# Joao-M-Silva/padel_analytics

Measured on AMD Instinct MI355X. Metric: frames/sec (all trackers) on 1280x720, higher is better.
Workload: dtype f32-equivalent (h2: fp16 pairs h + m/2048, 2 or 3 f16 MFMA products per multiply, fp32 accumulate)

## Files before the change

### padel_analytics_amd/csrc/engine.cpp

```cpp
#include "../../include/padel_hip.h"
#include "kernels.h"
#include <rccl/rccl.h>

#include <algorithm>
#include <cmath>
#include <cstdio>
#include <cstdlib>
#include <cstring>
#include <dlfcn.h>
#include <map>
#include <string>
#include <vector>

using namespace padel;

static thread_local std::string g_err;

struct Tuning {
    int impl = 2;
    int variant = -1;
    int tune = 1;
    int tap_pd = 2;
    int graph = 0;
    int timeline = 0;
    int alias = 1;
    int fuse_stem = 1;
    int w_single = 1;
    int fuse_sppf = 1;
    int fold_up = 1;
};

struct pa_comm;

struct pa_engine {
    int dev = 0;
    hipStream_t stream = nullptr;
    hipStream_t copy_stream = nullptr;
    std::string err;
    bool profiling = false;
    float* zeros = nullptr;
    Tuning t;
    int tuning_epoch = 0;
    std::string timeline_path;
    pa_comm* comm = nullptr;
};

static int env_int(const char* k, int dflt) { const char* v = getenv(k); return v ? atoi(v) : dflt; }

#define PA_FAIL(eng, ...)                                        \
    do {                                                         \
        char _b[512];                                            \
        snprintf(_b, sizeof(_b), __VA_ARGS__);                   \
        if (eng) (eng)->err = _b; else g_err = _b;               \
        return 1;                                                \
    } while (0)

#define PA_HIP(eng, call)                                                                  \
    do {                                                                                   \
        hipError_t _e = (call);                                                            \
        if (_e != hipSuccess) {                                                            \
            (void)hipGetLastError();    \
            PA_FAIL(eng, "%s failed: %s (%s:%d)", #call, hipGetErrorString(_e), __FILE__, __LINE__); \
        }                                                                                  \
    } while (0)

struct ProfRec { int kind; int ksize; double flops; hipEvent_t e0, e1; float ms; int M, cout, cin, stride, mf, nf, res; int tile; const char* family; };

struct pa_model {
    pa_engine* e = nullptr;
    pa_model_desc d{};
    std::vector<pa_buf_desc> bufs;
    std::vector<pa_op_desc> ops;
    std::vector<int> fold_src;
    std::vector<int> fold_dst;
    float* d_w = nullptr;
    size_t n_w = 0;
    char* d_wr = nullptr;
    std::vector<long long> wr_off;
    bool wr_valid = false;
    unsigned* d_ovf = nullptr;
    float* d_stage = nullptr; size_t stage_cap = 0;
    float* d_fc = nullptr;
    int fc_nout = 0;
    int max_batch = 64;

    bool planned = false;
    int p_h0 = 0, p_w0 = 0, p_imgsz = 0, p_pre = 0, p_auto = 0, p_batch = 0;
    int net_h = 0, net_w = 0;
    int rw = 0, rh = 0, top = 0, left = 0, lb_mode = 0;
    std::vector<float*> bptr;
    void* arena = nullptr;
    size_t arena_bytes = 0, logical_bytes = 0;
    unsigned h_ovf = 0;
    bool ovf_cached = false;
    unsigned* h_pin = nullptr;
    hipEvent_t tk_ev[PA_MAX_INFLIGHT]{};
    bool tk_busy[PA_MAX_INFLIGHT]{};
    int next_ticket = 0, n_inflight = 0;
    std::vector<int32_t> classes_host;
    std::map<int, hipGraphExec_t> graphs;
    int graph_epoch = -1;
    uint8_t* d_frames = nullptr; size_t frames_cap = 0;
    uint8_t* d_netin = nullptr;
    uint8_t* d_tmp = nullptr;
    int32_t *d_xtab = nullptr, *d_ytab = nullptr;
    int32_t *d_hb = nullptr, *d_hk = nullptr, *d_vb = nullptr, *d_vk = nullptr;
    int hks = 0, vks = 0;
    int A = 0, P2 = 0;
    HeadLevel lv[3]{};
    float* d_cand = nullptr; int32_t* d_cidx = nullptr; int32_t* d_ccnt = nullptr;
    uint64_t* d_keys = nullptr; int32_t* d_order = nullptr; uint8_t* d_supp = nullptr;
    float* d_oboxes = nullptr; float* d_okpts = nullptr; int32_t* d_ocnt = nullptr;
    int32_t* d_classes = nullptr; int classes_cap = 0;
    int last_n = 0;
    std::vector<ProfRec> prof;
    size_t n_prof = 0;
};

static void find_upsample_folds(pa_model* m);

extern "C" {

int pa_abi_version(void) { return PA_ABI_VERSION; }

int pa_device_count(void) {
    int n = 0;
    if (hipGetDeviceCount(&n) != hipSuccess) return 0;
    return n;
}

const char* pa_last_error(pa_engine* eng) { return eng ? eng->err.c_str() : g_err.c_str(); }

int pa_engine_create(int device_id, pa_engine** out) {
    if (!out) PA_FAIL((pa_engine*)nullptr, "pa_engine_create: out is NULL");
    int n = 0;
    PA_HIP((pa_engine*)nullptr, hipGetDeviceCount(&n));
    if (device_id < 0 || device_id >= n) PA_FAIL((pa_engine*)nullptr, "pa_engine_create: device %d of %d", device_id, n);
    PA_HIP((pa_engine*)nullptr, hipSetDevice(device_id));
    pa_engine* e = new pa_engine();
    e->dev = device_id;
    hipError_t r = hipStreamCreateWithFlags(&e->stream, hipStreamNonBlocking);
    if (r != hipSuccess) { delete e; PA_FAIL((pa_engine*)nullptr, "hipStreamCreate: %s", hipGetErrorString(r)); }
    if (r == hipSuccess) r = hipStreamCreateWithFlags(&e->copy_stream, hipStreamNonBlocking);
    if (r != hipSuccess) { delete e; PA_FAIL((pa_engine*)nullptr, "hipStreamCreate: %s", hipGetErrorString(r)); }
    r = hipMalloc((void**)&e->zeros, 256);
    if (r == hipSuccess) r = hipMemset(e->zeros, 0, 256);
    if (r != hipSuccess) { delete e; PA_FAIL((pa_engine*)nullptr, "zero page: %s", hipGetErrorString(r)); }
    r = padel::init_misc_kernels();
    if (r != hipSuccess) { delete e; PA_FAIL((pa_engine*)nullptr, "kernel attributes: %s", hipGetErrorString(r)); }
    if (const char* v = getenv("PADEL_CONV_IMPL")) {
        if (v[0] == 'l') { delete e; PA_FAIL((pa_engine*)nullptr, "PADEL_CONV_IMPL=%s: the LDS kernel was retired in round 5; tap or bx3", v); }
        e->t.impl = (v[0] == 'b') ? 2 : 0;
    }
    e->t.variant = env_int("PADEL_CONV_VARIANT", -1);
    e->t.tune = env_int("PADEL_CONV_TUNE", 1);
    e->t.tap_pd = env_int("PADEL_CONV_TAP_PD", 2) == 3 ? 3 : 2;
    e->t.graph = env_int("PADEL_GRAPH", 0);
    e->t.fuse_stem = env_int("PADEL_FUSE_STEM", 1);
    e->t.fuse_sppf = env_int("PADEL_FUSE_SPPF", 1);
    e->t.alias = env_int("PADEL_ALIAS", 1);
    e->t.fold_up = env_int("PADEL_FOLD_UP", 1);
    *out = e;
    return 0;
}

int pa_engine_set_tuning(pa_engine* e, const char* key, int value) {
    if (!e || !key) return 1;
    const std::string k = key;
    if (k == "impl") {
        if (value != 0 && value != 2) PA_FAIL(e, "tuning impl = %d: 0 (fp32-input MFMA tap kernels) or 2 (bf16x3); 1 was the LDS kernel, retired in round 5 (tools/legacy_conv)", value);
        e->t.impl = value;
    }
    else if (k == "variant") e->t.variant = value;
    else if (k == "tune") e->t.tune = value;
    else if (k == "tap_pd") e->t.tap_pd = (value == 3) ? 3 : 2;
    else if (k == "graph") e->t.graph = value ? 1 : 0;
    else if (k == "timeline") e->t.timeline = value ? 1 : 0;
    else if (k == "alias") e->t.alias = value ? 1 : 0;
    else if (k == "fold_up") e->t.fold_up = value ? 1 : 0;
    else if (!strcmp(key, "fuse_stem")) e->t.fuse_stem = value;
    else if (!strcmp(key, "fuse_sppf")) e->t.fuse_sppf = value;
    else if (!strcmp(key, "w_single")) e->t.w_single = value ? 1 : 0;
    else PA_FAIL(e, "pa_engine_set_tuning: unknown key '%s'", key);
    e->tuning_epoch++;
    return 0;
}

int pa_engine_set_timeline_path(pa_engine* e, const char* path) {
    if (!e) return 1;
    e->timeline_path = path ? path : "";
    return 0;
}

void pa_engine_destroy(pa_engine* e) {
    if (!e) return;
    hipSetDevice(e->dev);
    pa_engine_comm_destroy(e);
    if (e->zeros) hipFree(e->zeros);
    if (e->stream) hipStreamDestroy(e->stream);
    if (e->copy_stream) hipStreamDestroy(e->copy_stream);
    delete e;
}

int pa_engine_synchronize(pa_engine* e) {
    PA_HIP(e, hipSetDevice(e->dev));
    PA_HIP(e, hipStreamSynchronize(e->stream));
    return 0;
}

int pa_engine_set_profiling(pa_engine* e, int enable) { e->profiling = enable != 0; return 0; }

int pa_device_malloc(pa_engine* e, size_t nbytes, void** out) {
    PA_HIP(e, hipSetDevice(e->dev));
    PA_HIP(e, hipMalloc(out, nbytes));
    return 0;
}
int pa_device_free(pa_engine* e, void* p) {
    PA_HIP(e, hipSetDevice(e->dev));
    PA_HIP(e, hipFree(p));
    return 0;
}
int pa_memcpy_h2d(pa_engine* e, void* dst, const void* src, size_t n) {
    PA_HIP(e, hipSetDevice(e->dev));
    PA_HIP(e, hipMemcpyAsync(dst, src, n, hipMemcpyHostToDevice, e->stream));
    PA_HIP(e, hipStreamSynchronize(e->stream));
    return 0;
}
int pa_upload(pa_engine* e, void* dst, const void* src, size_t n) {
    PA_HIP(e, hipSetDevice(e->dev));
    PA_HIP(e, hipMemcpyAsync(dst, src, n, hipMemcpyHostToDevice, e->copy_stream));
    PA_HIP(e, hipStreamSynchronize(e->copy_stream));
    return 0;
}
int pa_host_register(pa_engine* e, void* ptr, size_t nbytes) {
    PA_HIP(e, hipSetDevice(e->dev));
    PA_HIP(e, hipHostRegister(ptr, nbytes, hipHostRegisterDefault));
    return 0;
}
int pa_host_unregister(pa_engine* e, void* ptr) {
    PA_HIP(e, hipSetDevice(e->dev));
    PA_HIP(e, hipHostUnregister(ptr));
    return 0;
}
int pa_memcpy_d2h(pa_engine* e, void* dst, const void* src, size_t n) {
    PA_HIP(e, hipSetDevice(e->dev));
    PA_HIP(e, hipMemcpyAsync(dst, src, n, hipMemcpyDeviceToHost, e->stream));
    PA_HIP(e, hipStreamSynchronize(e->stream));
    return 0;
}

static int validate_desc(pa_engine* e, const pa_model_desc* d, size_t n_floats) {
    if (d->n_bufs <= 0 || d->n_ops <= 0 || !d->bufs || !d->ops) PA_FAIL(e, "model desc: empty graph");
    const bool f16 = d->dtype == PA_DTYPE_F16, h2 = d->dtype == PA_DTYPE_H2;
    if (d->dtype != PA_DTYPE_F32 && d->dtype != PA_DTYPE_F16 && d->dtype != PA_DTYPE_H2) PA_FAIL(e, "model desc: dtype %d", d->dtype);
    const int kalign = f16 ? 31 : 15, valign = f16 ? 7 : 3;
    for (int i = 0; i < d->n_bufs; ++i)
        if (d->bufs[i].level < 0 || d->bufs[i].level > 6 || d->bufs[i].channels <= 0 || (d->bufs[i].channels & 3))
            PA_FAIL(e, "model desc: buffer %d (level %d, channels %d)", i, d->bufs[i].level, d->bufs[i].channels);
    auto okslice = [&](int b, int off, int c) {
        return b >= 0 && b < d->n_bufs && off >= 0 && c > 0 && off + c <= d->bufs[b].channels;
    };
    auto is_head_buf = [&](int b) { return b == d->head_buf[0] || b == d->head_buf[1] || b == d->head_buf[2]; };
    if (h2)
        for (int i = 0; i < d->n_bufs; ++i)
// ... 419 lines not shown
    return 0;
}

static ProfRec* prof_begin(pa_model* m, size_t idx, int kind, int ksize, double flops) {
    if (!m->e->profiling) return nullptr;
    if (m->prof.size() <= idx) {
        m->prof.resize(idx + 1);
        hipEventCreate(&m->prof[idx].e0);
        hipEventCreate(&m->prof[idx].e1);
    }
    ProfRec* r = &m->prof[idx];
    r->kind = kind; r->ksize = ksize; r->flops = flops; r->ms = 0.f;
    r->M = r->cout = r->cin = r->stride = r->mf = r->nf = r->res = 0;
    r->tile = -1; r->family = "";
    hipEventRecord(r->e0, m->e->stream);
    return r;
}
static void prof_end(pa_model* m, ProfRec* r) { if (r) hipEventRecord(r->e1, m->e->stream); }

static int conv_launch_args(const pa_model* m, size_t i, int n, ConvArgs& a) {
    const pa_engine* e = m->e;
    const pa_op_desc& o = m->ops[i];
    const pa_buf_desc& ob = m->bufs[o.out_buf];
    const pa_buf_desc& ib = m->bufs[o.in_buf];
    const int Ho = m->net_h >> ob.level, Wo = m->net_w >> ob.level;
    a.in = m->bptr[o.in_buf]; a.in_cs = ib.channels; a.in_choff = o.in_choff;
    a.out = m->bptr[o.out_buf]; a.out_cs = ob.channels; a.out_choff = o.out_choff;
    a.res = o.res_buf >= 0 ? m->bptr[o.res_buf] : nullptr;
    a.res_cs = o.res_buf >= 0 ? m->bufs[o.res_buf].channels : 0; a.res_choff = o.res_choff;
    a.res_pre = (o.res_buf >= 0 && (o.flags & PA_CONV_RES_PREACT)) ? 1 : 0;
    a.zeros = e->zeros;
    a.w = m->d_w + o.w_off; a.bias = m->d_w + o.b_off;
    a.H = m->net_h >> ib.level; a.W = m->net_w >> ib.level; a.Ho = Ho; a.Wo = Wo;
    a.cin = o.cin; a.cout = o.cout; a.n16 = o.npad / 16; a.ksize = o.ksize; a.stride = o.stride; a.act = o.act;
    a.M = n * Ho * Wo;
    fill_fastdiv((unsigned)(Ho * Wo), &a.howo_magic, &a.howo_shift);
    fill_fastdiv((unsigned)Wo, &a.wo_magic, &a.wo_shift);
    a.tune = e->t.tune; a.tap_pd = e->t.tap_pd;
    const bool f16 = m->d.dtype == PA_DTYPE_F16, h2 = m->d.dtype == PA_DTYPE_H2;
    const bool use_tap = e->t.impl == 0 || f16;
    const bool use_bx3 = !f16 && !h2 && e->t.impl == 2 && o.reserved > 0;
    a.w3 = use_bx3 ? (const void*)(m->d_w + o.reserved) : nullptr;
    a.out_f32 = (f16 || h2) && (o.out_buf == m->d.head_buf[0] || o.out_buf == m->d.head_buf[1] || o.out_buf == m->d.head_buf[2]);
    if (h2) {
        a.oscale = m->d_w + o.reserved;
        a.ovf_flag = m->d_ovf;
        a.w_single = (o.flags & PA_CONV_W_SINGLE) && e->t.w_single ? 1 : 0;
        a.wr = (m->wr_valid && i < m->wr_off.size() && m->wr_off[i] >= 0) ? (const void*)(m->d_wr + m->wr_off[i]) : nullptr;
        const int lv = e->t.variant >= 0 ? e->t.variant : choose_conv_h2_variant(a);
        if (fold_active(m, (int)i) && (o.ksize == 1 || (lv >= 300 && lv < 400 && conv_h2p_supported(a)))) {
            const pa_op_desc& u = m->ops[m->fold_src[i]];
            a.in2 = m->bptr[u.in_buf]; a.in2_cs = m->bufs[u.in_buf].channels; a.in2_choff = u.in_choff; a.up_c = u.cin;
        }
        return lv;
    }
    const int lv = e->t.variant >= 0 ? e->t.variant
                   : f16 ? choose_conv_tap16_variant(a)
                   : use_bx3 ? choose_conv_bx3_variant(a)
                         : choose_conv_tap_variant(a.M, a.n16);
    if (use_bx3 && fold_active(m, (int)i) && (o.ksize == 1 || (lv >= 300 && lv < 400 && conv_bx3p_supported(a)))) {
        const pa_op_desc& u = m->ops[m->fold_src[i]];
        a.in2 = m->bptr[u.in_buf]; a.in2_cs = m->bufs[u.in_buf].channels; a.in2_choff = u.in_choff; a.up_c = u.cin;
    }
    return lv;
}

static bool stem_fusable(const pa_model* m, size_t i) {
    if (i + 1 >= m->ops.size()) return false;
    const pa_op_desc& st = m->ops[i];
    const pa_op_desc& c = m->ops[i + 1];
    if (c.kind != PA_OP_CONV || c.ksize != 3 || c.stride != 2 || c.in_buf != st.out_buf || c.in_choff != st.out_choff || c.cin != st.cout ||
        c.res_buf >= 0)
        return false;
    for (int l = 0; l < 3; ++l) if (m->d.head_buf[l] == st.out_buf) return false;
    for (size_t k = 0; k < m->ops.size(); ++k) {
        if (k == i || k == i + 1) continue;
        const pa_op_desc& o = m->ops[k];
        if (o.kind != PA_OP_STEM && o.in_buf == st.out_buf) return false;
        if (o.kind == PA_OP_CONV && o.res_buf == st.out_buf) return false;
    }
    return true;
}

static int run_ops(pa_model* m, int n, size_t* pi) {
    pa_engine* e = m->e;
    hipStream_t s = e->stream;
    for (size_t i = 0; i < m->ops.size(); ++i) {
        const pa_op_desc& o = m->ops[i];
        const pa_buf_desc& ob = m->bufs[o.out_buf];
        const int Ho = m->net_h >> ob.level, Wo = m->net_w >> ob.level;
        hipError_t r = hipSuccess;
        ProfRec* pr = nullptr;
        if (o.kind == PA_OP_CONV) {
            ConvArgs a{};
            const int lv = conv_launch_args(m, i, n, a);
            const bool f16 = m->d.dtype == PA_DTYPE_F16, h2 = m->d.dtype == PA_DTYPE_H2;
            const bool use_tap = e->t.impl == 0 || f16;
            const bool use_bx3 = a.w3 != nullptr;
            int bm = 0, bn = 0;
            if (h2 && (lv == 323 || lv == 324)) { bm = 128; bn = 96; }
            else if (h2 && lv == 325) { bm = 128; bn = 64; }
            else if (h2 && lv == 244) { bm = 128; bn = 96; }
            else if (h2 && (lv == 245 || lv == 246)) { bm = 128; bn = 192; }
            else if (h2 && (lv == 247 || lv == 248)) { bm = 64; bn = 192; }
            else if (h2 && lv >= 341 && lv <= 343) { bm = 256; bn = (lv - 340) * 16; }
            else if (h2 && (lv == 243 || lv == 239)) conv_variant_shape(lv - 230, &bm, &bn);
            else if ((f16 || h2) && lv >= 300) { bm = 128; bn = ((lv - 300) % 10) * 16; }
            else if (f16) conv_tap16_variant_shape(lv, &bm, &bn);
            else if (lv >= 300) { bm = 128; bn = (lv - 300) * 16; }
            else conv_variant_shape(lv >= 200 ? lv - 200 : lv, &bm, &bn);
            pr = prof_begin(m, (*pi)++, o.kind, o.ksize, 2.0 * a.M * (double)o.cout * o.cin * o.ksize * o.ksize);
            if (pr) { pr->M = a.M; pr->cout = o.cout; pr->cin = o.cin; pr->stride = o.stride; pr->mf = bm; pr->nf = bn; pr->res = a.res != nullptr; }
            unsigned long long* dbg_dev = nullptr;
            size_t dbg_bytes = 0;
            if (e->t.timeline && h2 && ((lv == 323 && conv_h2q_supported(a)) || (lv == 324 && conv_h2r_supported(a))) && !e->timeline_path.empty()) {
                const size_t patches = (size_t)n * ((a.Ho + 7) / 8) * ((a.Wo + 15) / 16);
                dbg_bytes = 8 * ((patches + 7) / 8) * (size_t)((a.n16 + 5) / 6) * (8 + 4 * 32 * 5) * 8;
            } else if (e->t.timeline && !h2 && use_tap && lv == 7 && o.ksize == 3 && !e->timeline_path.empty()) {
                dbg_bytes = (size_t)((a.M + 63) / 64) * ((o.npad + 95) / 96) * kConvDbgWords * 8;
            }
            if (dbg_bytes) {
                if (hipMalloc(&dbg_dev, dbg_bytes) == hipSuccess) (void)hipMemsetAsync(dbg_dev, 0, dbg_bytes, s);
                else dbg_dev = nullptr;
                a.dbg = dbg_dev;
            }
            ConvLaunched ran{-1, ""};
            if (a.res_pre && !h2 && !use_bx3)
                PA_FAIL(e, "op %zu: PA_CONV_RES_PREACT needs the h2 or the bf16x3 kernels (tuning impl = 2, bf16x3 weights in the blob), not the %s family",
                        i, f16 ? "fp16" : "fp32-MFMA tap");
            if (h2) {
                r = launch_conv_h2(a, lv, s, &ran);
            } else if (f16) {
                r = launch_conv_tap16(a, lv, s, &ran);
            } else if (use_bx3) {
                r = launch_conv_bx3(a, lv, s, &ran);
            } else {
                r = launch_conv_tap(a, lv, s, &ran);
            }
            if (pr) { pr->tile = ran.tile; pr->family = ran.family; }
            if (dbg_dev) {
                (void)hipStreamSynchronize(s);
                std::vector<unsigned long long> host(dbg_bytes / 8);
                (void)hipMemcpy(host.data(), dbg_dev, dbg_bytes, hipMemcpyDeviceToHost);
                if (FILE* f = fopen(e->timeline_path.c_str(), "wb")) { fwrite(host.data(), 1, dbg_bytes, f); fclose(f); }
                (void)hipFree(dbg_dev);
            }
        } else if (o.kind == PA_OP_STEM) {
            StemArgs a{};
            a.in = m->d_netin; a.w = m->d_w + o.w_off; a.bias = m->d_w + o.b_off;
            a.out = m->bptr[o.out_buf]; a.out_cs = ob.channels; a.out_choff = o.out_choff;
            a.H = m->net_h; a.W = m->net_w; a.Ho = Ho; a.Wo = Wo; a.cout = o.cout; a.B = n;
            a.out_f16 = m->d.dtype == PA_DTYPE_F16 ? 1 : m->d.dtype == PA_DTYPE_H2 ? 2 : 0;
            a.ovf_flag = m->d_ovf;
            pr = prof_begin(m, (*pi)++, o.kind, 3, 2.0 * n * Ho * Wo * (double)o.cout * 27);
            if (e->t.fuse_stem && m->d.dtype == PA_DTYPE_H2 && stem_fusable(m, i)) {
                ConvArgs ca{};
                conv_launch_args(m, i + 1, n, ca);
                if (stem_l1_h2_supported(a, ca)) {
                    r = launch_stem_l1_h2(a, ca, s);
                    prof_end(m, pr);
                    if (r != hipSuccess) PA_FAIL(e, "fused stem + layer 1 launch failed: %s", hipGetErrorString(r));
                    ++i;
                    continue;
                }
            }
            r = launch_stem(a, s);
        } else if (o.kind == PA_OP_SPPF_POOL) {
            pr = prof_begin(m, (*pi)++, o.kind, 5, 0.0);
            r = launch_sppf_pool(m->bptr[o.in_buf], m->bufs[o.in_buf].channels, o.in_choff, o.cin, n, Ho, Wo, s, (int)m->d.dtype, e->t.fuse_sppf);
        } else if (o.kind == PA_OP_UPSAMPLE2X) {
            if (m->fold_dst[i] >= 0) {
                ConvArgs ca{};
                conv_launch_args(m, (size_t)m->fold_dst[i], n, ca);
                if (ca.in2) continue;
            }
            pr = prof_begin(m, (*pi)++, o.kind, 0, 0.0);
            r = launch_upsample2x(m->bptr[o.in_buf], m->bufs[o.in_buf].channels, o.in_choff, m->bptr[o.out_buf],
                                  ob.channels, o.out_choff, o.cin, n, Ho / 2, Wo / 2, s, (int)m->d.dtype);
        } else if (o.kind == PA_OP_MAXPOOL2) {
            pr = prof_begin(m, (*pi)++, o.kind, 2, 0.0);
            r = launch_maxpool2(m->bptr[o.in_buf], m->bufs[o.in_buf].channels, o.in_choff, m->bptr[o.out_buf],
                                ob.channels, o.out_choff, o.cin, n, Ho * 2, Wo * 2, s, (int)m->d.dtype);
        } else if (o.kind == PA_OP_MAXPOOL3S2) {
            const int lin = m->bufs[o.in_buf].level;
            pr = prof_begin(m, (*pi)++, o.kind, 3, 0.0);
            r = launch_maxpool3s2(m->bptr[o.in_buf], m->bufs[o.in_buf].channels, o.in_choff, m->bptr[o.out_buf], ob.channels, o.out_choff,
                                  o.cin, n, m->net_h >> lin, m->net_w >> lin, Ho, Wo, s, m->d.dtype == PA_DTYPE_H2 ? 1 : 0);
        } else if (o.kind == PA_OP_STEM7) {
            if (!m->d_netin) PA_FAIL(e, "op %zu: the 7x7 stem reads the u8 network input of pa_resnet_infer", i);
            const bool head = o.out_buf == m->d.head_buf[0] || o.out_buf == m->d.head_buf[1] || o.out_buf == m->d.head_buf[2];
            Stem7Args a{};
            a.in = m->d_netin; a.w = m->d_w + o.w_off; a.bias = m->d_w + o.b_off; a.lut = m->d_w + o.reserved;
            a.out = m->bptr[o.out_buf]; a.out_cs = ob.channels; a.out_choff = o.out_choff;
// ... 1058 lines not shown
```

### padel_analytics_amd/csrc/kernels.h

```cpp
#pragma once
#include <hip/hip_runtime.h>
#include <stdint.h>

namespace padel {

enum Act : int { ACT_NONE = 0, ACT_SILU = 1, ACT_RELU = 2, ACT_SIGMOID = 3, ACT_LEAKY = 4 };

struct ConvArgs {
    const float* in;
    const float* w;
    const void* w3;
    const float* bias;
    const float* res;
    int res_pre;
    const float* zeros;
    const float* in2;
    int in2_cs, in2_choff, up_c;
    float* out;
    int in_cs, in_choff;
    int out_cs, out_choff;
    int res_cs, res_choff;
    int H, W;
    int Ho, Wo;
    int cin;
    int cout;
    int n16;
    int ksize, stride;
    int act;
    int M;
    int n_mtiles;
    int n_ntiles;
    int tune;
    int tap_pd;
    int out_f32;
    const float* oscale;
    unsigned* ovf_flag;
    int w_single;
    const void* wr;
    unsigned long long* dbg;
    unsigned howo_magic, howo_shift, wo_magic, wo_shift;
};
inline void fill_fastdiv(unsigned d, unsigned* magic, unsigned* shift) {
    unsigned s = 0;
    while ((1ull << s) < d) ++s;
    *magic = (unsigned)((((1ull << 32) * ((1ull << s) - d)) / d) + 1ull);
    *shift = s;
}
constexpr int kConvDbgSteps = 64;
constexpr int kConvDbgWords = 8 + 4 * kConvDbgSteps * 5;

bool conv_variant_shape(int variant, int* bm, int* bn);
struct ConvLaunched { int tile; const char* family; };
inline hipError_t conv_ran(ConvLaunched* ran, int tile, const char* family, hipError_t e) {
    if (ran && e == hipSuccess) { ran->tile = tile; ran->family = family; }
    return e;
}
hipError_t launch_conv_tap(const ConvArgs& a, int variant, hipStream_t s, ConvLaunched* ran = nullptr);
constexpr size_t kConvReadSlack = 512;
int choose_conv_tap_variant(int M, int n16);
hipError_t launch_conv_bx3(const ConvArgs& a, int variant, hipStream_t s, ConvLaunched* ran = nullptr);
int choose_conv_bx3_variant(const ConvArgs& a);
bool conv_bx3p_supported(const ConvArgs& a);
hipError_t launch_conv_bx3p(const ConvArgs& a, int nf, hipStream_t s);
hipError_t launch_conv_h2(const ConvArgs& a, int variant, hipStream_t s, ConvLaunched* ran = nullptr);
int choose_conv_h2_variant(const ConvArgs& a);
bool conv_h2p_supported(const ConvArgs& a);
hipError_t launch_conv_h2p(const ConvArgs& a, int nf, hipStream_t s);
bool conv_h2q_supported(const ConvArgs& a);
hipError_t launch_conv_h2q(const ConvArgs& a, hipStream_t s);
bool conv_h2r_supported(const ConvArgs& a);
hipError_t launch_conv_h2r(const ConvArgs& a, int nf, hipStream_t s);
size_t conv_h2r_copy_bytes(int n16, int cin, int ksize);
hipError_t launch_h2r_repack(const float* w, void* wr, int n16, int cin, int ksize, hipStream_t s);
bool conv_h2s_supported(const ConvArgs& a);
hipError_t launch_conv_h2s(const ConvArgs& a, bool nf12, hipStream_t s, bool m64 = false);
bool conv_h2s3_supported(const ConvArgs& a);
hipError_t launch_conv_h2s3(const ConvArgs& a, hipStream_t s, bool m64 = false);
hipError_t launch_h2_mplane_check(const float* w, long long rows_x_ksteps, unsigned* flag, hipStream_t s);
hipError_t launch_conv_h2_deep(const ConvArgs& a, int variant, hipStream_t s);
bool conv_h2w_supported(const ConvArgs& a);
hipError_t launch_conv_h2w(const ConvArgs& a, int nf, hipStream_t s);
bool conv_h2v_supported(const ConvArgs& a);
hipError_t launch_conv_h2v(const ConvArgs& a, int nf, hipStream_t s);
hipError_t launch_conv_tap16(const ConvArgs& a, int variant, hipStream_t s, ConvLaunched* ran = nullptr);
int choose_conv_tap16_variant(const ConvArgs& a);
bool conv_tap16_variant_shape(int variant, int* bm, int* bn);
bool conv_p16_supported(const ConvArgs& a);
hipError_t launch_conv_p16(const ConvArgs& a, int nf, hipStream_t s);

struct StemArgs {
    const uint8_t* in;
    const float* w;
    const float* bias;
    float* out;
    int out_cs, out_choff;
    int H, W, Ho, Wo, cout, B;
    int out_f16;
    unsigned* ovf_flag;
    unsigned howo_magic, howo_shift, wo_magic, wo_shift;
};
hipError_t launch_stem(const StemArgs& a, hipStream_t s);
struct ConvArgs;
bool stem_l1_h2_supported(const StemArgs& st, const ConvArgs& cv);
hipError_t launch_stem_l1_h2(const StemArgs& st, const ConvArgs& cv, hipStream_t s);

hipError_t init_misc_kernels();
hipError_t launch_sppf_pool(float* buf, int cs, int choff, int c, int B, int H, int W, hipStream_t s, int f16 = 0, int fused = 1);
hipError_t launch_upsample2x(const float* in, int in_cs, int in_choff, float* out, int out_cs, int out_choff,
                             int c, int B, int H, int W, hipStream_t s, int f16 = 0);
hipError_t launch_h2_encode(const float* in, float* out, long long n_floats, unsigned* ovf_flag, hipStream_t s);
hipError_t launch_maxpool2(const float* in, int in_cs, int in_choff, float* out, int out_cs, int out_choff,
                           int c, int B, int H, int W, hipStream_t s, int f16 = 0);

struct Stem7Args {
    const uint8_t* in;
    const float* w;
    const float* bias;
    const float* lut;
    float* out;
    int out_cs, out_choff;
    int H, W, Ho, Wo, B;
    int act;
    int out_h2;
    unsigned* ovf_flag;
    unsigned howo_magic, howo_shift, wo_magic, wo_shift;
};
hipError_t launch_stem7(const Stem7Args& a, hipStream_t s);
hipError_t launch_maxpool3s2(const float* in, int in_cs, int in_choff, float* out, int out_cs, int out_choff,
                             int c, int B, int H, int W, int Ho, int Wo, hipStream_t s, int h2);
hipError_t launch_gap_fc(const float* in, int in_cs, int in_choff, int c, int B, int HW, const float* w, const float* bias, int nout,
                         float* logits, float* probs, hipStream_t s, int h2);
constexpr int kGapFcMaxC = 4096, kGapFcMaxOut = 64;

struct LetterboxArgs {
    const uint8_t* src;
    uint8_t* dst;
    int B, h0, w0;
    int rw, rh;
    int top, left;
    int nh, nw;
    int mode;
    int reverse;
    const int32_t* xtab;
    const int32_t* ytab;
};
hipError_t launch_letterbox(const LetterboxArgs& a, hipStream_t s);

struct ResamplePassArgs {
    const uint8_t* in; uint8_t* out;
    int B, in_h, in_w, in_c;
    int out_h, out_w, out_c;
    int vertical;
    const int32_t* bounds;
    const int32_t* coefs;
    int ksize;
    int reverse;
};
hipError_t launch_resample_pass(const ResamplePassArgs& a, hipStream_t s);

struct HeadLevel { const float* buf; int H, W, stride, anchor0; };
struct DecodeArgs {
    HeadLevel lv[3];
    int cs;
    int nc, nk, kdim;
    int A, B;
    float conf;
// ... 59 lines not shown
```

Before: 1014.

## Fuse consecutive 3x3 bottleneck conv pairs into one h2 kernel with LDS intermediate

Adds a kernel that runs two back-to-back 3x3 stride-1 convolutions (cin=cout=16/32/48) in one launch. The first conv computes an 18x18 halo tile from a 20x20 input patch held in LDS, encodes the intermediate to h2 in registers, and feeds it to the second conv without a global-memory round trip. The engine detects fusable pairs, checking that the intermediate buffer is not read elsewhere, and falls back to the separate launches otherwise. This removes one launch and the intermediate write/read per pair, at the cost of recomputing the halo and heavier register and LDS use per workgroup.

```diff
diff --git a/padel_analytics_amd/csrc/conv_patch_h2vv.hip b/padel_analytics_amd/csrc/conv_patch_h2vv.hip
--- /dev/null
+++ b/padel_analytics_amd/csrc/conv_patch_h2vv.hip
@@ -0,0 +1,428 @@
+#include "h2_common.h"
+
+namespace padel {
+
+namespace {
+
+constexpr int kMW = 18, kMNPix = 18 * 18;
+constexpr int kMSpans = (kMNPix + 15) / 16;
+constexpr int kMPlaneB = kMSpans * 1024;
+constexpr int kMTSpans = (kMNPix + 31) / 32;
+constexpr int kMTPlaneB = kMTSpans * 1024;
+constexpr int kIW = 20, kINPix = 20 * 20;
+constexpr int kISpans = (kINPix + 15) / 16;
+constexpr int kIPlaneB = kISpans * 1024;
+constexpr int kITSpans = (kINPix + 31) / 32;
+constexpr int kITPlaneB = kITSpans * 1024;
+
+__device__ __forceinline__ unsigned vv_swz64(unsigned t) { return t ^ ((t >> 3) & 32u); }
+__device__ __forceinline__ unsigned vv_swz32(unsigned u) { return u ^ ((u >> 4) & 16u); }
+
+typedef int vv_i32x4 __attribute__((ext_vector_type(4)));
+
+template <int ACT, int NF>
+__device__ __forceinline__ void vv_mid_encode(const f32x4 (&mainacc)[3][NF], const f32x4 (&cross)[3][NF], const f32x4 (&b)[NF],
+                                              const f32x4 (&sc)[NF], const bool (&inimg)[3], const bool (&own)[3],
+                                              h2_u32x2 (&mh)[3][NF], h2_u32x2 (&mm)[3][NF], h2_u16x2& top, bool& bad_slow) {
+#pragma unroll
+    for (int j = 0; j < NF; ++j)
+#pragma unroll
+        for (int f = 0; f < 3; ++f) {
+            f32x4 v;
+#pragma unroll
+            for (int r = 0; r < 4; ++r) v[r] = h2_act<ACT>(h2_conv_value(cross[f][j][r], mainacc[f][j][r], sc[j][r], b[j][r]));
+            const unsigned keep = inimg[f] ? 0xFFFFFFFFu : 0u, chk = own[f] ? 0x7FFF7FFFu : 0u;
+#pragma unroll
+            for (int p = 0; p < 2; ++p) {
+                bad_slow = bad_slow || (own[f] && (!(fabsf(v[2 * p]) <= kH2Max) || !(fabsf(v[2 * p + 1]) <= kH2Max)));
+                const h2_f32x2 x = {__builtin_amdgcn_fmed3f(v[2 * p], -kH2Max, kH2Max), __builtin_amdgcn_fmed3f(v[2 * p + 1], -kH2Max, kH2Max)};
+                const h2_h16x2 hh = __builtin_convertvector(x, h2_h16x2);
+                const h2_f32x2 res = {(x[0] - (float)hh[0]) * kH2Scale, (x[1] - (float)hh[1]) * kH2Scale};
+                const h2_h16x2 mmv = __builtin_convertvector(res, h2_h16x2);
+                const unsigned hd = __builtin_bit_cast(unsigned, hh), md = __builtin_bit_cast(unsigned, mmv);
+                top = __builtin_elementwise_max(top, __builtin_bit_cast(h2_u16x2, hd & chk));
+                mh[f][j][p] = hd & keep;
+                mm[f][j][p] = md & keep;
+            }
+        }
+}
+
+}
+
+template <int C>
+__global__ void __launch_bounds__(256, 2) conv_h2vv_kernel(const ConvArgs a1, const ConvArgs a2) {
+    static_assert(C == 16 || C == 32 || C == 48, "cin = cout = 16 / 32 / 48");
+    constexpr bool CHUNK = C >= 32, TAIL = (C & 16) != 0;
+    constexpr int NF = C / 16;
+    constexpr int MF = 4, MF1 = 3;
+    constexpr int NSTEPS = (CHUNK ? 9 : 0) + (TAIL ? 5 : 0);
+    constexpr int IN_CB = CHUNK ? 2 * kIPlaneB : 0;
+    constexpr int IN_B = IN_CB + (TAIL ? 2 * kITPlaneB : 0);
+    constexpr int PATCH_B = CHUNK ? 2 * kMPlaneB : 0;
+    constexpr int MID_B = PATCH_B + (TAIL ? 2 * kMTPlaneB : 0);
+    static_assert(MID_B <= IN_B && IN_B <= 80 * 1024, "the intermediate overlays the input patch; 2 workgroups per CU");
+    __shared__ __attribute__((aligned(16))) float lds[IN_B / 4];
+    char* const ldsb = reinterpret_cast<char*>(lds);
+    const int tid = threadIdx.x;
+    const int lane = tid & 63;
+    const int wave = __builtin_amdgcn_readfirstlane(tid >> 6);
+    const int lr = lane & 15, lq = lane >> 4;
+
+    const int nmt = a2.n_mtiles;
+    const int bid = blockIdx.x;
+    const int q8 = nmt >> 3, r8 = nmt & 7, xcd = bid & 7, mloc = bid >> 3;
+    if (mloc >= q8 + (xcd < r8 ? 1 : 0)) return;
+    const int mt = (xcd < r8 ? xcd * (q8 + 1) : r8 * (q8 + 1) + (xcd - r8) * q8) + mloc;
+    const int txN = (a2.Wo + 15) >> 4, tyN = (a2.Ho + 15) >> 4;
+    const int tpi = tyN * txN;
+    const int n = mt / tpi, rt = mt - n * tpi;
+    const int ty = rt / txN, tx = rt - ty * txN;
+    const int y0 = ty * 16, x0 = tx * 16;
+
+    const float* const in0 = a1.in + (((long long)n * a1.H + (y0 - 2)) * a1.W + (x0 - 2)) * a1.in_cs + a1.in_choff;
+    const i32x4 rsrcP = make_rsrc3(in0);
+    const unsigned lp0 = __builtin_amdgcn_readfirstlane((unsigned)(uintptr_t)lds);
+
+    if constexpr (CHUNK) {
+        const int p_lane = lane >> 2;
+        const int p_q = (lane & 3) ^ (((lane >> 4) & 1) << 1);
+        const unsigned p_piece = (unsigned)((p_q >> 1) * 64 + (p_q & 1) * 16);
+        for (int sp = wave; sp < kISpans; sp += 4) {
+            const int pp = sp * 16 + p_lane;
+            const int py = pp / kIW, px = pp - py * kIW;
+            const bool ok = (unsigned)(y0 - 2 + py) < (unsigned)a1.H && (unsigned)(x0 - 2 + px) < (unsigned)a1.W;
+            const unsigned vo = ok ? (unsigned)((py * a1.W + px) * a1.in_cs * 4) + p_piece : kOOR3;
+            const unsigned la = __builtin_amdgcn_readfirstlane(lp0 + (unsigned)sp * 1024u);
+            dma3<0>(vo, rsrcP, 0u, la);
+            dma3<kIPlaneB>(vo, rsrcP, 32u, la);
+        }
+    }
+    if constexpr (TAIL) {
+        const int t_lane = lane >> 1;
+        const unsigned t_piece = (unsigned)(((lane & 1) ^ ((lane >> 4) & 1)) * 16);
+        const unsigned t_so = CHUNK ? 128u : 0u;
+        for (int sp = (wave + 1) & 3; sp < kITSpans; sp += 4) {
+            const int pp = sp * 32 + t_lane;
+            const int py = pp / kIW, px = pp - py * kIW;
+            const bool ok = pp < kINPix && (unsigned)(y0 - 2 + py) < (unsigned)a1.H && (unsigned)(x0 - 2 + px) < (unsigned)a1.W;
+            const unsigned vo = ok ? (unsigned)((py * a1.W + px) * a1.in_cs * 4) + t_piece : kOOR3;
+            const unsigned la = __builtin_amdgcn_readfirstlane(lp0 + (unsigned)(IN_CB + sp * 1024));
+            dma3<0>(vo, rsrcP, t_so, la);
+            dma3<kITPlaneB>(vo, rsrcP, t_so + 32u, la);
+        }
+    }
+
+    constexpr unsigned fragb = (unsigned)NSTEPS * 2048u;
+    const unsigned voffW = (unsigned)lane * 16u;
+    i32x4 rsrcW1[NF], rsrcW2[NF];
+#pragma unroll
+    for (int j = 0; j < NF; ++j) {
+        rsrcW1[j] = make_rsrc3(reinterpret_cast<const char*>(a1.wr) + (long long)j * fragb);
+        rsrcW2[j] = make_rsrc3(reinterpret_cast<const char*>(a2.wr) + (long long)j * fragb);
+    }
+    vv_i32x4 w[3][NF];
+#define PADEL_VV_LOADW(RS_, ST_)                                                                                  \
+    do {                                                                                                          \
+        const unsigned so_ = (unsigned)((ST_) * 2048);                                                            \
+        _Pragma("unroll") for (int j = 0; j < NF; ++j)                                                            \
+            asm volatile("buffer_load_dwordx4 %0, %1, %2, %3 offen"                                               \
+                         : "=v"(w[(ST_) % 3][j]) : "v"(voffW), "s"(RS_[j]), "s"(so_) : "memory");                 \
+    } while (0)
+#define PADEL_VV_WAITW(ST_, N_)                                                                                   \
+    do {                                                                                                          \
+        if constexpr (NF == 3)                                                                                    \
+            asm volatile("s_waitcnt vmcnt(%3)" : "+v"(w[(ST_) % 3][0]), "+v"(w[(ST_) % 3][1]), "+v"(w[(ST_) % 3][NF - 1]) : "n"(N_) : "memory"); \
+        else if constexpr (NF == 2)                                                                               \
+            asm volatile("s_waitcnt vmcnt(%2)" : "+v"(w[(ST_) % 3][0]), "+v"(w[(ST_) % 3][NF - 1]) : "n"(N_) : "memory"); \
+        else                                                                                                      \
+            asm volatile("s_waitcnt vmcnt(%1)" : "+v"(w[(ST_) % 3][0]) : "n"(N_) : "memory");                     \
+    } while (0)
+#define PADEL_VV_TOP(RS_, ST_)                                                                                    \
+    do {                                                                                                          \
+        if constexpr ((ST_) + 2 < NSTEPS) PADEL_VV_LOADW(RS_, (ST_) + 2);                                         \
+        PADEL_VV_WAITW(ST_, NF * (((ST_) + 1 < NSTEPS ? 1 : 0) + ((ST_) + 2 < NSTEPS ? 1 : 0)));                  \
+        __builtin_amdgcn_sched_barrier(0);                                                                        \
+    } while (0)
+
+    PADEL_VV_LOADW(rsrcW1, 0);
+    PADEL_VV_LOADW(rsrcW1, 1);
+    wait_vm3<NF * 2>();
+    __builtin_amdgcn_s_barrier();
+    asm volatile("" ::: "memory");
+
+    h2_u32x2 mid_h[2][MF1][NF], mid_m[2][MF1][NF];
+    h2_u16x2 top1 = {0, 0};
+    bool bad_slow1 = false;
+    h16x8 ah[4], am[4];
+#pragma unroll
+    for (int P = 0; P < 2; ++P) {
+#define PADEL_VV1_LIVE(F_) ((F_) < 2 || P == 0 || wave == 0)
+        unsigned t0[MF1], u0[MF1];
+        bool inimg[MF1], own[MF1];
+#pragma unroll
+        for (int f = 0; f < MF1; ++f) {
+            const int q = (wave + 4 * (3 * P + f)) * 16 + lr;
+            const int qc = min(q, kMNPix - 1);
+            const int iy = qc / kMW, ix = qc - iy * kMW;
+            const int p0 = iy * kIW + ix;
+            t0[f] = (unsigned)(p0 * 64 + lq * 16);
+            u0[f] = (unsigned)(p0 * 32 + (lq & 1) * 16);
+            inimg[f] = q < kMNPix && (unsigned)(y0 - 1 + iy) < (unsigned)a1.H && (unsigned)(x0 - 1 + ix) < (unsigned)a1.W;
+            own[f] = inimg[f] && (unsigned)(iy - 1) < 16u && (unsigned)(ix - 1) < 16u;
+        }
+        f32x4 acc1[MF1][NF], part1[MF1][NF], cross1[MF1][NF];
+#pragma unroll
+        for (int f = 0; f < MF1; ++f)
+#pragma unroll
+            for (int j = 0; j < NF; ++j) { acc1[f][j] = (f32x4){0.f, 0.f, 0.f, 0.f}; part1[f][j] = acc1[f][j]; cross1[f][j] = acc1[f][j]; }
+#define PADEL_VV1_READ(F_, T_)                                                                                    \
+        do {                                                                                                      \
+            constexpr int d_ = h2_tap_ky(T_) * kIW + h2_tap_kx(T_);                                               \
+            const char* p_ = ldsb + vv_swz64(t0[F_] + (unsigned)(d_ * 64));                                       \
+            ah[F_] = *reinterpret_cast<const h16x8*>(p_);                                                         \
+            am[F_] = *reinterpret_cast<const h16x8*>(p_ + kIPlaneB);                                              \
+        } while (0)
+#define PADEL_VV1_MFMA(F_, ST_)                                                                                   \
+        do {                                                                                                      \
+            if (PADEL_VV1_LIVE(F_)) {                                                                             \
+                _Pragma("unroll") for (int j = 0; j < NF; ++j)                                                    \
+                    cross1[F_][j] = __builtin_amdgcn_mfma_f32_16x16x32_f16(__builtin_bit_cast(h16x8, w[(ST_) % 3][j]), am[F_], cross1[F_][j], 0, 0, 0); \
+                _Pragma("unroll") for (int j = 0; j < NF; ++j)                                                    \
+                    part1[F_][j] = __builtin_amdgcn_mfma_f32_16x16x32_f16(__builtin_bit_cast(h16x8, w[(ST_) % 3][j]), ah[F_], part1[F_][j], 0, 0, 0); \
+            }                                                                                                     \
+            __builtin_amdgcn_sched_barrier(0);                                                                    \
+        } while (0)
+#define PADEL_VV1_STEP(T_)                                                                                        \
+        do {                                                                                                      \
+            PADEL_VV_TOP(rsrcW1, T_);                                                                             \
+            PADEL_VV1_MFMA(0, T_);                                                                                \
+            if constexpr ((T_) < 8) PADEL_VV1_READ(0, (T_) + 1);                                                  \
+            __builtin_amdgcn_sched_barrier(0);                                                                    \
+            PADEL_VV1_MFMA(1, T_);                                                                                \
+            if constexpr ((T_) < 8) PADEL_VV1_READ(1, (T_) + 1);                                                  \
+            __builtin_amdgcn_sched_barrier(0);                                                                    \
+            PADEL_VV1_MFMA(2, T_);                                                                                \
+            if constexpr ((T_) < 8) PADEL_VV1_READ(2, (T_) + 1);                                                  \
+            __builtin_amdgcn_sched_barrier(0);                                                                    \
+        } while (0)
+#define PADEL_VV1_TSTEP(JT_, ST_)                                                                                 \
+        do {                                                                                                      \
+            constexpr int ta_ = 2 * (JT_), tb_ = 2 * (JT_) + 1 < 9 ? 2 * (JT_) + 1 : 8;                           \
+            constexpr unsigned da_ = (unsigned)((h2_tap_ky(ta_) * kIW + h2_tap_kx(ta_)) * 32);                    \
+            constexpr unsigned db_ = (unsigned)((h2_tap_ky(tb_) * kIW + h2_tap_kx(tb_)) * 32);                    \
+            const unsigned dd_ = (lq >> 1) ? db_ : da_;                                                           \
+            _Pragma("unroll") for (int f = 0; f < MF1; ++f) {                                                     \
+                const char* p_ = ldsb + IN_CB + vv_swz32(u0[f] + dd_);                                            \
+                ah[f] = *reinterpret_cast<const h16x8*>(p_);                                                      \
+                am[f] = *reinterpret_cast<const h16x8*>(p_ + kITPlaneB);                                          \
+            }                                                                                                     \
+            __builtin_amdgcn_sched_barrier(0);                                                                    \
+            PADEL_VV_TOP(rsrcW1, ST_);                                                                            \
+            PADEL_VV1_MFMA(0, ST_); PADEL_VV1_MFMA(1, ST_); PADEL_VV1_MFMA(2, ST_);                               \
+        } while (0)
+#define PADEL_VV1_FLUSH()                                                                                         \
+        do {                                                                                                      \
+            _Pragma("unroll") for (int f = 0; f < MF1; ++f)                                                       \
+                _Pragma("unroll") for (int j = 0; j < NF; ++j) { acc1[f][j] += part1[f][j]; part1[f][j] = (f32x4){0.f, 0.f, 0.f, 0.f}; } \
+        } while (0)
+        if (P == 1) {
+            PADEL_VV_LOADW(rsrcW1, 0);
+            PADEL_VV_LOADW(rsrcW1, 1);
+        }
+        if constexpr (CHUNK) {
+            PADEL_VV1_READ(0, 0); PADEL_VV1_READ(1, 0); PADEL_VV1_READ(2, 0);
+            __builtin_amdgcn_sched_barrier(0);
+            PADEL_VV1_STEP(0); PADEL_VV1_STEP(1); PADEL_VV1_STEP(2); PADEL_VV1_STEP(3); PADEL_VV1_STEP(4);
+            PADEL_VV1_STEP(5); PADEL_VV1_STEP(6); PADEL_VV1_STEP(7); PADEL_VV1_STEP(8);
+            PADEL_VV1_FLUSH();
+        }
+        if constexpr (TAIL) {
+            constexpr int S0 = CHUNK ? 9 : 0;
+            PADEL_VV1_TSTEP(0, S0); PADEL_VV1_TSTEP(1, S0 + 1); PADEL_VV1_TSTEP(2, S0 + 2); PADEL_VV1_TSTEP(3, S0 + 3); PADEL_VV1_TSTEP(4, S0 + 4);
+            PADEL_VV1_FLUSH();
+        }
+#undef PADEL_VV1_FLUSH
+#undef PADEL_VV1_TSTEP
+#undef PADEL_VV1_STEP
+#undef PADEL_VV1_MFMA
+#undef PADEL_VV1_READ
+#undef PADEL_VV1_LIVE
+        f32x4 b1[NF], sc1[NF];
+#pragma unroll
+        for (int j = 0; j < NF; ++j) {
+            b1[j] = *reinterpret_cast<const f32x4*>(a1.bias + j * 16 + lq * 4);
+            sc1[j] = *reinterpret_cast<const f32x4*>(a1.oscale + j * 16 + lq * 4);
+        }
+        if (a1.act == ACT_SILU) vv_mid_encode<ACT_SILU, NF>(acc1, cross1, b1, sc1, inimg, own, mid_h[P], mid_m[P], top1, bad_slow1);
+        else if (a1.act == ACT_RELU) vv_mid_encode<ACT_RELU, NF>(acc1, cross1, b1, sc1, inimg, own, mid_h[P], mid_m[P], top1, bad_slow1);
+        else if (a1.act == ACT_SIGMOID) vv_mid_encode<ACT_SIGMOID, NF>(acc1, cross1, b1, sc1, inimg, own, mid_h[P], mid_m[P], top1, bad_slow1);
+        else if (a1.act == ACT_LEAKY) vv_mid_encode<ACT_LEAKY, NF>(acc1, cross1, b1, sc1, inimg, own, mid_h[P], mid_m[P], top1, bad_slow1);
+        else vv_mid_encode<ACT_NONE, NF>(acc1, cross1, b1, sc1, inimg, own, mid_h[P], mid_m[P], top1, bad_slow1);
+        asm volatile("" ::: "memory");
+    }
+    {
+        const bool fast1 = y0 + 16 <= a1.Ho && x0 + 16 <= a1.Wo && (((a1.out_choff | a1.out_cs) & 15) == 0);
+        h2_raise(a1.ovf_flag, fast1 ? (top1[0] >= 0x7BFFu || top1[1] >= 0x7BFFu) : bad_slow1);
+    }
+
+    __builtin_amdgcn_s_barrier();
+    asm volatile("" ::: "memory");
+    PADEL_VV_LOADW(rsrcW2, 0);
+    PADEL_VV_LOADW(rsrcW2, 1);
+#pragma unroll
+    for (int P = 0; P < 2; ++P)
+#pragma unroll
+        for (int f = 0; f < MF1; ++f) {
+            const int q = (wave + 4 * (3 * P + f)) * 16 + lr;
+            if (q < kMNPix) {
+#pragma unroll
+                for (int j = 0; j < NF; ++j) {
+                    char* p_;
+                    if (CHUNK && j < 2) p_ = ldsb + vv_swz64((unsigned)(q * 64 + (2 * j + (lq >> 1)) * 16)) + (lq & 1) * 8;
+                    else p_ = ldsb + PATCH_B + vv_swz32((unsigned)(q * 32 + (lq >> 1) * 16)) + (lq & 1) * 8;
+                    *reinterpret_cast<h2_u32x2*>(p_) = mid_h[P][f][j];
+                    *reinterpret_cast<h2_u32x2*>(p_ + ((CHUNK && j < 2) ? kMPlaneB : kMTPlaneB)) = mid_m[P][f][j];
+                }
+            }
+        }
+    asm volatile("s_waitcnt lgkmcnt(0)" ::: "memory");
+    __builtin_amdgcn_s_barrier();
+    asm volatile("" ::: "memory");
+
+    unsigned rbase[8];
+    if constexpr (CHUNK) {
+#pragma unroll
+        for (int r = 0; r < 8; ++r) {
+            const int p0 = 4 * wave * kMW + lr;
+            rbase[r] = (unsigned)(p0 * 64 + ((lq ^ ((((p0 + r) >> 2) & 1) << 1)) << 4));
+        }
+    }
+    const int rd_pix = 4 * wave * kMW + lr;
+
+    f32x4 acc[MF][NF], part[MF][NF], cross[MF][NF];
+#pragma unroll
+    for (int f = 0; f < MF; ++f)
+#pragma unroll
+        for (int j = 0; j < NF; ++j) { acc[f][j] = (f32x4){0.f, 0.f, 0.f, 0.f}; part[f][j] = acc[f][j]; cross[f][j] = acc[f][j]; }
+#define PADEL_VV_READROW(R_, KX_)                                                                                 \
+    do {                                                                                                          \
+        constexpr int d_ = (R_) * kMW + (KX_);                                                                    \
+        const char* p_ = ldsb + rbase[d_ & 7];                                                                    \
+        ah[(R_) & 3] = *reinterpret_cast<const h16x8*>(p_ + d_ * 64);                                             \
+        am[(R_) & 3] = *reinterpret_cast<const h16x8*>(p_ + d_ * 64 + kMPlaneB);                                  \
+    } while (0)
+#define PADEL_VV_MFMA_ROW(F_, S_, ST_)                                                                            \
+    do {                                                                                                          \
+        _Pragma("unroll") for (int j = 0; j < NF; ++j)                                                            \
+            cross[F_][j] = __builtin_amdgcn_mfma_f32_16x16x32_f16(__builtin_bit_cast(h16x8, w[(ST_) % 3][j]), am[S_], cross[F_][j], 0, 0, 0); \
+        _Pragma("unroll") for (int j = 0; j < NF; ++j)                                                            \
+            part[F_][j] = __builtin_amdgcn_mfma_f32_16x16x32_f16(__builtin_bit_cast(h16x8, w[(ST_) % 3][j]), ah[S_], part[F_][j], 0, 0, 0); \
+        __builtin_amdgcn_sched_barrier(0);                                                                        \
+    } while (0)
+#define PADEL_VV_STEP(T_)                                                                                         \
+    do {                                                                                                          \
+        constexpr int kx_ = h2_tap_kx(T_), ky_ = h2_tap_ky(T_);                                                   \
+        PADEL_VV_TOP(rsrcW2, T_);                                                                                 \
+        if constexpr (ky_ == 0) {                                                                                 \
+            PADEL_VV_MFMA_ROW(0, 0, T_);                                                                          \
+            PADEL_VV_READROW(4, kx_);                                                                             \
+            __builtin_amdgcn_sched_barrier(0);                                                                    \
+            PADEL_VV_MFMA_ROW(1, 1, T_); PADEL_VV_MFMA_ROW(2, 2, T_); PADEL_VV_MFMA_ROW(3, 3, T_);                \
+        } else if constexpr (ky_ == 1) {                                                                          \
+            PADEL_VV_MFMA_ROW(0, 1, T_);                                                                          \
+            PADEL_VV_READROW(5, kx_);                                                                             \
+            __builtin_amdgcn_sched_barrier(0);                                                                    \
+            PADEL_VV_MFMA_ROW(1, 2, T_); PADEL_VV_MFMA_ROW(2, 3, T_); PADEL_VV_MFMA_ROW(3, 0, T_);                \
+        } else {                                            \
+            PADEL_VV_MFMA_ROW(2, 0, T_);                                                                          \
+            if constexpr (kx_ < 2) PADEL_VV_READROW(0, kx_ + 1);                                                  \
+            __builtin_amdgcn_sched_barrier(0);                                                                    \
+            PADEL_VV_MFMA_ROW(3, 1, T_);                                                                          \
+            if constexpr (kx_ < 2) PADEL_VV_READROW(1, kx_ + 1);                                                  \
+            __builtin_amdgcn_sched_barrier(0);                                                                    \
+            PADEL_VV_MFMA_ROW(0, 2, T_);                                                                          \
+            if constexpr (kx_ < 2) PADEL_VV_READROW(2, kx_ + 1);                                                  \
+            __builtin_amdgcn_sched_barrier(0);                                                                    \
+            PADEL_VV_MFMA_ROW(1, 3, T_);                                                                          \
+            if constexpr (kx_ < 2) PADEL_VV_READROW(3, kx_ + 1);                                                  \
+            __builtin_amdgcn_sched_barrier(0);                                                                    \
+        }                                                                                                         \
+    } while (0)
+#define PADEL_VV_TSTEP(JT_, ST_)                                                                                  \
+    do {                                                                                                          \
+        constexpr int ta_ = 2 * (JT_), tb_ = 2 * (JT_) + 1 < 9 ? 2 * (JT_) + 1 : 8;                               \
+        int rp_ = rd_pix;                                                                                         \
+        asm volatile("" : "+v"(rp_));                                                                             \
+        _Pragma("unroll") for (int f = 0; f < MF; ++f) {                                                          \
+            const int pa_ = rp_ + (f + h2_tap_ky(ta_)) * kMW + h2_tap_kx(ta_), pb_ = rp_ + (f + h2_tap_ky(tb_)) * kMW + h2_tap_kx(tb_); \
+            const int pp_ = (lq >> 1) ? pb_ : pa_;                                                                \
+            const char* p_ = ldsb + PATCH_B + vv_swz32((unsigned)(pp_ * 32 + (lq & 1) * 16));                     \
+            ah[f] = *reinterpret_cast<const h16x8*>(p_);                                                          \
+            am[f] = *reinterpret_cast<const h16x8*>(p_ + kMTPlaneB);                                              \
+        }                                                                                                         \
+        __builtin_amdgcn_sched_barrier(0);                                                                        \
+        PADEL_VV_TOP(rsrcW2, ST_);                                                                                \
+        PADEL_VV_MFMA_ROW(0, 0, ST_); PADEL_VV_MFMA_ROW(1, 1, ST_); PADEL_VV_MFMA_ROW(2, 2, ST_); PADEL_VV_MFMA_ROW(3, 3, ST_); \
+    } while (0)
+#define PADEL_VV_FLUSH()                                                                                          \
+    do {                                                                                                          \
+        _Pragma("unroll") for (int f = 0; f < MF; ++f)                                                            \
+            _Pragma("unroll") for (int j = 0; j < NF; ++j) { acc[f][j] += part[f][j]; part[f][j] = (f32x4){0.f, 0.f, 0.f, 0.f}; } \
+    } while (0)
+    if constexpr (CHUNK) {
+        PADEL_VV_READROW(0, 0); PADEL_VV_READROW(1, 0); PADEL_VV_READROW(2, 0); PADEL_VV_READROW(3, 0);
+        __builtin_amdgcn_sched_barrier(0);
+        PADEL_VV_STEP(0); PADEL_VV_STEP(1); PADEL_VV_STEP(2); PADEL_VV_STEP(3); PADEL_VV_STEP(4);
+        PADEL_VV_STEP(5); PADEL_VV_STEP(6); PADEL_VV_STEP(7); PADEL_VV_STEP(8);
+        PADEL_VV_FLUSH();
+    }
+    if constexpr (TAIL) {
+        constexpr int S0 = CHUNK ? 9 : 0;
+        PADEL_VV_TSTEP(0, S0); PADEL_VV_TSTEP(1, S0 + 1); PADEL_VV_TSTEP(2, S0 + 2); PADEL_VV_TSTEP(3, S0 + 3); PADEL_VV_TSTEP(4, S0 + 4);
+        PADEL_VV_FLUSH();
+    }
+#undef PADEL_VV_FLUSH
+#undef PADEL_VV_TSTEP
+#undef PADEL_VV_STEP
+#undef PADEL_VV_MFMA_ROW
+#undef PADEL_VV_READROW
+#undef PADEL_VV_TOP
+#undef PADEL_VV_WAITW
+#undef PADEL_VV_LOADW
+
+    int mpix[MF];
+#pragma unroll
+    for (int f = 0; f < MF; ++f) {
+        const int oy = y0 + 4 * wave + f, ox = x0 + lr;
+        mpix[f] = (oy < a2.Ho && ox < a2.Wo) ? (n * a2.Ho + oy) * a2.Wo + ox : -1;
+    }
+    const bool fast = y0 + 16 <= a2.Ho && x0 + 16 <= a2.Wo && (((a2.out_choff | a2.out_cs) & 3) == 0) &&
+                      (!a2.res || (((a2.res_choff | a2.res_cs) & 3) == 0));
+    h2_epilogue<MF, NF>(a2, acc, cross, mpix, 0, lq, fast);
+}
+
+bool conv_h2vv_supported(const ConvArgs& a1, const ConvArgs& a2) {
+    if (!conv_h2v_supported(a1) || !conv_h2v_supported(a2)) return false;
+    if (!a1.w_single || !a2.w_single || a1.res || a1.out_f32 || a2.out_f32) return false;
+    const int c = a1.cin;
+    if (a1.cout != c || a2.cin != c || a2.cout != c || a1.n16 * 16 != c || a2.n16 * 16 != c) return false;
+    if (a1.H != a2.H || a1.W != a2.W || a1.M != a2.M) return false;
+    if (reinterpret_cast<const float*>(a1.out) != a2.in || a1.out_cs != a2.in_cs || a1.out_choff != a2.in_choff) return false;
+    if (!a1.oscale || !a2.oscale || !a1.bias || !a2.bias || !a1.ovf_flag || a1.ovf_flag != a2.ovf_flag) return false;
+    return true;
+}
+
+hipError_t launch_conv_h2vv(const ConvArgs& a1, const ConvArgs& a2_in, hipStream_t s) {
+    if (!conv_h2vv_supported(a1, a2_in)) return hipErrorNotSupported;
+    ConvArgs a2 = a2_in;
+    const int batch = a2.M / (a2.Ho * a2.Wo);
+    a2.n_mtiles = batch * ((a2.Ho + 15) / 16) * ((a2.Wo + 15) / 16);
+    a2.n_ntiles = 1;
+    dim3 grid(8u * (unsigned)((a2.n_mtiles + 7) / 8), 1, 1);
+    if (a2.cin == 48) hipLaunchKernelGGL((conv_h2vv_kernel<48>), grid, dim3(256), 0, s, a1, a2);
+    else if (a2.cin == 32) hipLaunchKernelGGL((conv_h2vv_kernel<32>), grid, dim3(256), 0, s, a1, a2);
+    else hipLaunchKernelGGL((conv_h2vv_kernel<16>), grid, dim3(256), 0, s, a1, a2);
+    return hipGetLastError();
+}
+
+}
diff --git a/padel_analytics_amd/csrc/engine.cpp b/padel_analytics_amd/csrc/engine.cpp
--- a/padel_analytics_amd/csrc/engine.cpp
+++ b/padel_analytics_amd/csrc/engine.cpp
@@ -27,6 +27,7 @@
     int fuse_stem = 1;
     int w_single = 1;
     int fuse_sppf = 1;
+    int fuse_pair = 1;
     int fold_up = 1;
 };
 
@@ -158,6 +159,7 @@
     e->t.graph = env_int("PADEL_GRAPH", 0);
     e->t.fuse_stem = env_int("PADEL_FUSE_STEM", 1);
     e->t.fuse_sppf = env_int("PADEL_FUSE_SPPF", 1);
+    e->t.fuse_pair = env_int("PADEL_FUSE_PAIR", 1);
     e->t.alias = env_int("PADEL_ALIAS", 1);
     e->t.fold_up = env_int("PADEL_FOLD_UP", 1);
     *out = e;
@@ -180,6 +182,7 @@
     else if (k == "fold_up") e->t.fold_up = value ? 1 : 0;
     else if (!strcmp(key, "fuse_stem")) e->t.fuse_stem = value;
     else if (!strcmp(key, "fuse_sppf")) e->t.fuse_sppf = value;
+    else if (!strcmp(key, "fuse_pair")) e->t.fuse_pair = value ? 1 : 0;
     else if (!strcmp(key, "w_single")) e->t.w_single = value ? 1 : 0;
     else PA_FAIL(e, "pa_engine_set_tuning: unknown key '%s'", key);
     e->tuning_epoch++;
@@ -765,6 +768,32 @@
     return true;
 }
 
+static bool pair_fusable(const pa_model* m, size_t i) {
+    const pa_engine* e = m->e;
+    if (!e->t.fuse_pair || !e->t.w_single || e->t.variant >= 0 || e->t.timeline || (e->t.tune & 8)) return false;
+    if (m->d.dtype != PA_DTYPE_H2 || i + 1 >= m->ops.size()) return false;
+    const pa_op_desc& o1 = m->ops[i];
+    const pa_op_desc& o2 = m->ops[i + 1];
+    const int c = o1.cin;
+    if (c != 16 && c != 32 && c != 48) return false;
+    for (const pa_op_desc* o : {&o1, &o2})
+        if (o->kind != PA_OP_CONV || o->ksize != 3 || o->stride != 1 || o->cin != c || o->cout != c || !(o->flags & PA_CONV_W_SINGLE)) return false;
+    if (o1.res_buf >= 0 || o2.in_buf != o1.out_buf || o2.in_choff != o1.out_choff || o2.res_buf == o1.out_buf) return false;
+    const int lv = m->bufs[o1.in_buf].level;
+    if (m->bufs[o1.out_buf].level != lv || m->bufs[o2.out_buf].level != lv) return false;
+    if (fold_active(m, (int)i) || fold_active(m, (int)i + 1)) return false;
+    for (int l = 0; l < 3; ++l) if (m->d.head_buf[l] == o1.out_buf || m->d.head_buf[l] == o2.out_buf) return false;
+    const size_t nops = m->ops.size();
+    for (size_t d = 2; d < nops; ++d) {
+        const pa_op_desc& o = m->ops[(i + d) % nops];
+        if (o.kind != PA_OP_STEM && o.kind != PA_OP_STEM7 && o.in_buf == o1.out_buf) return false;
+        if (o.kind == PA_OP_CONV && o.res_buf == o1.out_buf) return false;
+        if (o.kind == PA_OP_CONV && o.out_buf == o1.out_buf && o.out_choff <= o1.out_choff && o.out_choff + o.cout >= o1.out_choff + o1.cout) break;
+    }
+    return true;
+}
+static bool pair_tile_ok(int lv, const ConvArgs& a) { return lv >= 341 && lv <= 343 && a.n16 % (lv - 340) == 0 && !a.in2; }
+
 static int run_ops(pa_model* m, int n, size_t* pi) {
     pa_engine* e = m->e;
     hipStream_t s = e->stream;
@@ -792,6 +821,26 @@
             else if (f16) conv_tap16_variant_shape(lv, &bm, &bn);
             else if (lv >= 300) { bm = 128; bn = (lv - 300) * 16; }
             else conv_variant_shape(lv >= 200 ? lv - 200 : lv, &bm, &bn);
+            if (h2 && pair_tile_ok(lv, a) && pair_fusable(m, i)) {
+                ConvArgs a2{};
+                const int lv2 = conv_launch_args(m, i + 1, n, a2);
+                if (pair_tile_ok(lv2, a2) && conv_h2vv_supported(a, a2)) {
+                    const pa_op_desc& o2 = m->ops[i + 1];
+                    const double fl = 2.0 * a.M * 9.0 * ((double)o.cout * o.cin + (double)o2.cout * o2.cin);
+                    pr = prof_begin(m, *pi, o2.kind, 3, fl);
+                    if (pr) { pr->M = a2.M; pr->cout = o2.cout; pr->cin = o2.cin; pr->stride = 1; pr->mf = 256; pr->nf = o2.cout; pr->res = a2.res != nullptr; }
+                    r = launch_conv_h2vv(a, a2, s);
+                    if (r == hipSuccess) {
+                        if (pr) { pr->tile = 350 + o2.cout / 16; pr->family = "h2vv"; }
+                        prof_end(m, pr);
+                        ++(*pi);
+                        ++i;
+                        continue;
+                    }
+                    if (r != hipErrorNotSupported) PA_FAIL(e, "op %zu: fused bottleneck pair launch failed: %s", i, hipGetErrorString(r));
+                    r = hipSuccess;
+                }
+            }
             pr = prof_begin(m, (*pi)++, o.kind, o.ksize, 2.0 * a.M * (double)o.cout * o.cin * o.ksize * o.ksize);
             if (pr) { pr->M = a.M; pr->cout = o.cout; pr->cin = o.cin; pr->stride = o.stride; pr->mf = bm; pr->nf = bn; pr->res = a.res != nullptr; }
             unsigned long long* dbg_dev = nullptr;
diff --git a/padel_analytics_amd/csrc/kernels.h b/padel_analytics_amd/csrc/kernels.h
--- a/padel_analytics_amd/csrc/kernels.h
+++ b/padel_analytics_amd/csrc/kernels.h
@@ -82,6 +82,8 @@
 hipError_t launch_conv_h2w(const ConvArgs& a, int nf, hipStream_t s);
 bool conv_h2v_supported(const ConvArgs& a);
 hipError_t launch_conv_h2v(const ConvArgs& a, int nf, hipStream_t s);
+bool conv_h2vv_supported(const ConvArgs& a1, const ConvArgs& a2);
+hipError_t launch_conv_h2vv(const ConvArgs& a1, const ConvArgs& a2, hipStream_t s);
 hipError_t launch_conv_tap16(const ConvArgs& a, int variant, hipStream_t s, ConvLaunched* ran = nullptr);
 int choose_conv_tap16_variant(const ConvArgs& a);
 bool conv_tap16_variant_shape(int variant, int* bm, int* bn);
```

After: 1022 (median of 6 runs). Within noise of the previous version (+0.7%).
